# zhengfei0908/SBA-GAN

Hardware: AMD Instinct MI355X
Metric: images/sec (G+D step) at 256px (higher is better)
Workload: dtype bf16; 1 GPU; bird_style.yml 3-stage G+D step (64..256px), B=20 per GPU, G_NET variant=model, image_encoder=inception, text_encoder=RNN_ENCODER in the step; global_batch=20, parallelism=dp1, launch=replayer, losses_finite=True

## Files before the change

sba-gan_amd/csrc/igemm.hip:

```cpp
#include <math.h>
#include <stdlib.h>

#include "common.h"
#include <type_traits>

namespace {

struct FastDiv {
    uint64_t magic;
    uint32_t d;
};
static inline FastDiv make_fastdiv(uint32_t d, int64_t max_n) {
    FastDiv f;
    f.d = d;
    f.magic = (max_n < (1 << 21) && d > 0) ? (((uint64_t)1 << 42) + d - 1) / d : 0;
    return f;
}
__device__ __forceinline__ uint32_t fdiv(uint32_t n, const FastDiv& f) {
    return f.magic ? (uint32_t)(((uint64_t)n * f.magic) >> 42) : n / f.d;
}

struct EpiX { const float* bias; const void* mask; int yh; int glu_c; };

__device__ __forceinline__ uint32_t relu_mask_bf16x2(uint32_t v, uint32_t m) {
// ... 1877 lines not shown
        typedef __attribute__((address_space(3))) s16x4_t* lptr;
        s16x4_t lo = __builtin_amdgcn_ds_read_tr16_b64_v4i16((lptr)(xs + slot(L0) * 128 + c0 * 16 + q * 8));
        s16x4_t hi = __builtin_amdgcn_ds_read_tr16_b64_v4i16((lptr)(xs + slot(L1) * 128 + c1 * 16 + q * 8));
        bf16x8_t v;
        v[0] = lo[0]; v[1] = lo[1]; v[2] = lo[2]; v[3] = lo[3];
        v[4] = hi[0]; v[5] = hi[1]; v[6] = hi[2]; v[7] = hi[3];
        return v;
    }
};

template <int KW, int XB> struct WgRowCfg {
    static constexpr int LPS = (4 + XB + KW - 1) / KW;
    static constexpr int STAGE = LPS * KW * 1024;
};

template <int KW, int SX, int XB, int D>
__global__ __launch_bounds__(64 * KW, 2) void wgrad_row_dma_kernel(const bf16_t* __restrict__ x, const bf16_t* __restrict__ dy,
                                                                float* __restrict__ dw, const sba_conv_geom g, const int M,
                                                                const int chunks_per_split, const int use_atomic,
                                                                const FastDiv dsub, const FastDiv dow, const int64_t zstride,
                                                                const int wclog) {
    constexpr int LPS = WgRowCfg<KW, XB>::LPS, STAGE = WgRowCfg<KW, XB>::STAGE;
    extern __shared__ __attribute__((aligned(1024))) unsigned char wg_lds[];

    const int tid = threadIdx.x, lane = tid & 63, wv = __builtin_amdgcn_readfirstlane(tid >> 6);
    const int kw = wv;
    const int co0 = blockIdx.x * 64;
    const int ci_tiles = g.Cin / 64;
    const int kh = blockIdx.y / ci_tiles;
    const int ci0 = (blockIdx.y - kh * ci_tiles) * 64;
    const int tap = kh * KW + kw;
    int ty0 = 0, tx0 = 0;
#pragma unroll
    for (int t = 0; t < SBA_MAX_TAPS; ++t) {
        if (t == kh * KW) { ty0 = g.ty[t]; tx0 = g.tx[t]; }
    }
    const int ups = g.ups;
    const int Wc = 1 << wclog, R = 32 >> wclog, XW = ups ? (Wc >> 1) + 2 : SX * (Wc - 1) + KW, XR = R * XW;
    const int sub = g.OH * g.OW;

    const uint32_t lds_base = (uint32_t)(uintptr_t)(__attribute__((address_space(3))) unsigned char*)wg_lds;
    const uint32_t x_bytes = (uint32_t)((int64_t)g.N * g.IH * g.IW * g.Cin * 2);
    const uint32_t dy_bytes = (uint32_t)((int64_t)g.N * g.OH * g.OW * g.Cout * 2);
    const __amdgpu_buffer_rsrc_t xr = __builtin_amdgcn_make_buffer_rsrc((void*)x, 0, x_bytes, 0x00020000);
    const __amdgpu_buffer_rsrc_t dr = __builtin_amdgcn_make_buffer_rsrc((void*)dy, 0, dy_bytes, 0x00020000);
    constexpr uint32_t OOB = 0xFFFFFFFFu;

    const int rsub = lane >> 3;
    const int cgx = (lane & 7) ^ WgFragRow<SX>::swz(rsub);
    const int cgd = (lane & 7) ^ (((lane >> 4) & 1) << 2);
    const uint32_t x_coff = (uint32_t)(ci0 + cgx * 8) * 2u, d_coff = (uint32_t)(co0 + cgd * 8) * 2u;
    const uint32_t x_pix = (uint32_t)g.Cin * 2u, d_pix = (uint32_t)g.Cout * 2u;
    const int rows_img = g.OH < R ? g.OH : R;
    int role[LPS], rr[LPS], rc[LPS], rn[LPS];
#pragma unroll
    for (int i = 0; i < LPS; ++i) {
        const int b = wv + KW * i;
        role[i] = 2; rr[i] = 0; rc[i] = 0; rn[i] = 0;
        if (b < 4) { role[i] = 0; rr[i] = 8 * b + rsub; }
        else if (b < 4 + XB) {
            const int L = WgFragRow<SX>::slot(8 * (b - 4) + rsub);
            if (L < XR) {
                const int r = L / XW;
                role[i] = 1;
                rn[i] = r / rows_img;
                rr[i] = (r - rn[i] * rows_img) * g.sy + ty0;
                rc[i] = ups ? L - r * XW : L - r * XW + tx0;
            }
        }
    }

    const int chunk_lo = blockIdx.z * chunks_per_split;
    const int chunk_hi = min(chunk_lo + chunks_per_split, M >> 5);
    int g_ck = chunk_lo;

    auto issue = [&](const uint32_t dst) {
        const bool live = g_ck < chunk_hi;
        const int m0 = g_ck * 32;
        const int n = (int)fdiv(m0, dsub), rem = m0 - n * sub;
        const int oy0 = (int)fdiv(rem, dow), ox0 = rem - oy0 * g.OW;
        const int iy0 = oy0 * g.sy, ix0 = ox0 * g.sx;
#pragma unroll
        for (int i = 0; i < LPS; ++i) {
            uint32_t off = OOB;
            if (role[i] == 0) {
                if (live) off = (uint32_t)(m0 + rr[i]) * d_pix + d_coff;
                lds_dma16(dr, off, 0u, dst + (uint32_t)((wv + KW * i) * 1024));
            } else {
                int iy = iy0 + rr[i], ix = ix0 + rc[i];
                if (ups) {
                    iy >>= 1;
                    ix = ((ox0 + tx0) >> 1) + rc[i];
                }
                const bool ok = live & (role[i] == 1) & (iy >= 0) & (iy < g.IH) & (ix >= 0) & (ix < g.IW);
                if (ok) off = (uint32_t)(((n + rn[i]) * g.IH + iy) * g.IW + ix) * x_pix + x_coff;
                lds_dma16(xr, off, 0u, dst + (uint32_t)((wv + KW * i) * 1024));
            }
        }
        ++g_ck;
    };

    f32x16_t acc[2][2];
#pragma unroll
    for (int i = 0; i < 2; ++i)
#pragma unroll
        for (int j = 0; j < 2; ++j)
#pragma unroll
            for (int r = 0; r < 16; ++r) acc[i][j][r] = 0.f;

    int islot = 0;
#pragma unroll
    for (int p = 0; p < D - 1; ++p) { issue(lds_base + (uint32_t)(islot * STAGE)); ++islot; }
    if (islot == D) islot = 0;
    int cslot = 0;
    for (int ck = chunk_lo; ck < chunk_hi; ++ck) {
        wait_vmcnt<(D - 2) * LPS>();
        wg_barrier();
        issue(lds_base + (uint32_t)(islot * STAGE));
        if (++islot == D) islot = 0;
        const unsigned char* st = wg_lds + cslot * STAGE;
        const unsigned char* xs = st + 4 * 1024;
#pragma unroll
        for (int k16 = 0; k16 < 2; ++k16) {
            bf16x8_t a[2], b[2];
            b[0] = WgFragRow<SX>::load(xs, k16, 0, lane, kw, wclog, XW, ups, tx0);
            b[1] = WgFragRow<SX>::load(xs, k16, 32, lane, kw, wclog, XW, ups, tx0);
            a[0] = WgFragDma::load(st, k16, 0, lane);
            a[1] = WgFragDma::load(st, k16, 32, lane);
#pragma unroll
            for (int i = 0; i < 2; ++i)
#pragma unroll
                for (int j = 0; j < 2; ++j)
                    acc[i][j] = __builtin_amdgcn_mfma_f32_32x32x16_bf16(a[i], b[j], acc[i][j], 0, 0, 0);
        }
        if (++cslot == D) cslot = 0;
    }
    wait_vmcnt<0>();
    wg_barrier();

    const int col_l = lane & 31, rsel = 4 * (lane >> 5);
#pragma unroll
    for (int i = 0; i < 2; ++i)
#pragma unroll
        for (int j = 0; j < 2; ++j)
#pragma unroll
            for (int r = 0; r < 16; ++r) {
                const int co = co0 + i * 32 + (r & 3) + 8 * (r >> 2) + rsel;
                const int ci = ci0 + j * 32 + col_l;
                float* p = dw + (int64_t)blockIdx.z * zstride + ((int64_t)co * g.ntaps + tap) * g.Cin + ci;
                if (use_atomic == 1) atomicAdd(p, acc[i][j][r]);
                else if (use_atomic == 2) *p = acc[i][j][r];
                else *p += acc[i][j][r];
            }
}

template <typename T>
__global__ __launch_bounds__(192) void wgrad_rows_kernel(const T* __restrict__ x, const T* __restrict__ dy,
                                                         float* __restrict__ dw, const sba_conv_geom g,
                                                         const int total_segs, const int segs_per_wg,
                                                         const int store, const int64_t zstride) {
    constexpr int ROWS = WgFrag<T>::ROWS;
    constexpr int CH = 16 / (int)sizeof(T);
    constexpr int CPR = 64 / CH;
    constexpr int XR = 66;
    constexpr int XROWS_ALLOC = 80;
    __shared__ __attribute__((aligned(16))) unsigned char lds[(64 + 3 * XROWS_ALLOC) * ROWS];

    const int tid = threadIdx.x, lane = tid & 63, kh = tid >> 6;
    const int co0 = blockIdx.x * 64, ci0 = blockIdx.y * 64;
    const int IHL = g.ups ? 2 * g.IH : g.IH, IWL = g.ups ? 2 * g.IW : g.IW;
    const int segs_per_row = g.OW / 64;
    unsigned char* sa = lds;
    unsigned char* sx = lds + (64 + kh * XROWS_ALLOC) * ROWS;

    for (int i = lane; i < (XROWS_ALLOC - XR) * ROWS / 16; i += 64)
        *reinterpret_cast<uint4*>(sx + XR * ROWS + i * 16) = make_uint4(0, 0, 0, 0);

    f32x16_t acc[3][2][2];
#pragma unroll
    for (int t = 0; t < 3; ++t)
#pragma unroll
        for (int i = 0; i < 2; ++i)
#pragma unroll
            for (int j = 0; j < 2; ++j)
#pragma unroll
                for (int r = 0; r < 16; ++r) acc[t][i][j][r] = 0.f;

    const int seg_lo = blockIdx.z * segs_per_wg;
    const int seg_hi = min(seg_lo + segs_per_wg, total_segs);
    constexpr int A_PT = (64 * CPR + 191) / 192;
    constexpr int X_PT = (XR * CPR + 63) / 64;
    uint4 va[A_PT], vx[X_PT];
    auto gload = [&](int seg) {
        const int n = seg / (g.OH * segs_per_row);
        const int rem = seg - n * g.OH * segs_per_row;
        const int oy = rem / segs_per_row, ox0 = (rem - oy * segs_per_row) * 64;
#pragma unroll
        for (int u = 0; u < A_PT; ++u) {
            const int idx = tid + 192 * u;
            va[u] = make_uint4(0, 0, 0, 0);
            if (idx < 64 * CPR) {
                const int pix = idx / CPR, cc = idx - pix * CPR;
                const int co = co0 + cc * CH;
                if (co < g.Cout) {
                    const int64_t po = ((int64_t)(n * g.OH + oy) * g.OW + ox0 + pix);
                    va[u] = *reinterpret_cast<const uint4*>(dy + po * g.Cout + co);
                }
            }
        }
        int iy = oy + kh - 1;
        const bool row_ok = (iy >= 0) & (iy < IHL);
        if (g.ups) iy >>= 1;
#pragma unroll
        for (int u = 0; u < X_PT; ++u) {
            const int idx = lane + 64 * u;
            vx[u] = make_uint4(0, 0, 0, 0);
            if (idx < XR * CPR) {
                const int j = idx / CPR, cc = idx - j * CPR;
                int ix = ox0 - 1 + j;
                const bool ok = row_ok & (ix >= 0) & (ix < IWL);
                if (g.ups) ix >>= 1;
                const int ci = ci0 + cc * CH;
                if (ok && ci < g.Cin) {
                    const int64_t pi = (int64_t)(n * g.IH + iy) * g.IW + ix;
                    vx[u] = *reinterpret_cast<const uint4*>(x + pi * g.Cin + ci);
                }
            }
        }
    };
    if (seg_lo < seg_hi) gload(seg_lo);
    for (int seg = seg_lo; seg < seg_hi; ++seg) {
        __syncthreads();
#pragma unroll
        for (int u = 0; u < A_PT; ++u) {
            const int idx = tid + 192 * u;
            if (idx < 64 * CPR) {
                const int pix = idx / CPR, cc = idx - pix * CPR;
                *reinterpret_cast<uint4*>(sa + pix * ROWS + cc * 16) = va[u];
            }
        }
#pragma unroll
        for (int u = 0; u < X_PT; ++u) {
            const int idx = lane + 64 * u;
            if (idx < XR * CPR) {
                const int j = idx / CPR, cc = idx - j * CPR;
                *reinterpret_cast<uint4*>(sx + j * ROWS + cc * 16) = vx[u];
            }
        }
        __syncthreads();
        if (seg + 1 < seg_hi) gload(seg + 1);
#pragma unroll
        for (int ks = 0; ks < 4; ++ks) {
#pragma unroll
            for (int kw = 0; kw < 3; ++kw)
                WgFrag<T>::mma(sa + 16 * ks * ROWS, sx + (16 * ks + kw) * ROWS, lane, acc[kw]);
        }
    }

    const int col_l = lane & 31, rsel = 4 * (lane >> 5);
#pragma unroll
    for (int kw = 0; kw < 3; ++kw) {
        const int tap = kh * 3 + kw;
#pragma unroll
        for (int i = 0; i < 2; ++i)
#pragma unroll
            for (int j = 0; j < 2; ++j)
#pragma unroll
                for (int r = 0; r < 16; ++r) {
                    const int co = co0 + i * 32 + (r & 3) + 8 * (r >> 2) + rsel;
                    const int ci = ci0 + j * 32 + col_l;
                    if (co < g.Cout && ci < g.Cin) {
                        float* p = dw + (int64_t)blockIdx.z * zstride + ((int64_t)co * 9 + tap) * g.Cin + ci;
                        if (store) *p = acc[kw][i][j][r];
                        else atomicAdd(p, acc[kw][i][j][r]);
                    }
                }
    }
}

template <typename T>
__global__ void pack_weight_kernel(const float* __restrict__ w, T* __restrict__ out, int Cout, int KH,
                                   int KW, int Cin, int mode) {
    const int64_t n = (int64_t)Cout * (mode == 3 ? 16 : KH * KW) * Cin;
    for (int64_t i = blockIdx.x * (int64_t)blockDim.x + threadIdx.x; i < n;
         i += (int64_t)gridDim.x * blockDim.x) {
        float v;
        if (mode == 0) {
            v = w[i];
        } else if (mode == 1) {
            const int co = (int)(i % Cout);
            int64_t t = i / Cout;
            const int kw = (int)(t % KW); t /= KW;
            const int kh = (int)(t % KH);
            const int ci = (int)(t / KH);
            v = w[(((int64_t)co * KH + (KH - 1 - kh)) * KW + (KW - 1 - kw)) * Cin + ci];
        } else if (mode == 3) {
            const int co = (int)(i % Cout);
            int64_t t = i / Cout;
            const int sl = (int)(t % 16);
            const int ci = (int)(t / 16);
            const int dd = sl >> 2, ee = sl & 3;
            const int kh0 = dd == 0 ? 2 : (dd == 1 ? 1 : 0), khn = (dd == 1 || dd == 2) ? 2 : 1;
            const int kw0 = ee == 0 ? 2 : (ee == 1 ? 1 : 0), kwn = (ee == 1 || ee == 2) ? 2 : 1;
            v = 0.f;
            for (int a = 0; a < khn; ++a)
                for (int b2 = 0; b2 < kwn; ++b2)
// ... 213 lines not shown
            if (sizeof(T) == 2 && ex.yh) *reinterpret_cast<bf16_t*>(&ov[k]) = f2h_bits(v[k]);
            else ov[k] = from_f<T>(v[k]);
        }
        *reinterpret_cast<V4*>(y + o) = *reinterpret_cast<const V4*>(ov);
    }
    if (stats) {
        float* slot = stats + (int64_t)(blockIdx.y & (SBA_BN_STAT_SLOTS - 1)) * 2 * g.Cout;
#pragma unroll
        for (int k = 0; k < 4; ++k) {
            atomicAdd(&slot[c + k], s0[k]);
            atomicAdd(&slot[g.Cout + c + k], s1[k]);
        }
    }
}

template <typename T>
__global__ __launch_bounds__(256) void splitk_finish_kernel(float* __restrict__ ws, T* __restrict__ y,
                                                            const T* __restrict__ addend,
                                                            float* __restrict__ stats, const sba_conv_geom g,
                                                            const int M, const EpiX ex) {
    splitk_finish_body<T>(ws, y, addend, stats, g, M, ex);
}

__global__ __launch_bounds__(256) void splitk_finish_group_kernel(const GroupArgs A) {
    const GroupItem& it = A.it[blockIdx.z];
    const sba_conv_geom g = it.g;
    splitk_finish_body<bf16_t>(it.ws, it.y, it.addend, nullptr, g, it.M, EpiX{it.bias, it.mask, 0});
}

struct IgemmCfg { int bm, bn, ks, occ; float eff; bool split; };
static const IgemmCfg kCfg[5] = {
    {128, 128, 1, 3, 1.00f, false}, {256, 64, 1, 3, 1.00f, false}, {128, 64, 2, 2, 0.80f, false},
    {64, 64, 2, 4, 0.50f, true},    {320, 128, 2, 1, 0.90f, true}};
constexpr int IGEMM_SPLIT_MAX_M = 2048;

template <typename T, int BM, int BN, int WM, int WN, int KS>
static void launch_cfg(const T* xp, const T* wp, T* yp, const T* ap, float* stats, const sba_conv_geom& g, int M,
                       int nslabs, int split, float* ws, hipStream_t st, const EpiX ex) {
    constexpr int NT = (BM / WM) * (BN / WN) * 64;
    int sps = nslabs;
    if (split > 1) {
        sps = cdiv(cdiv(nslabs, split), KS) * KS;
        split = cdiv(nslabs, sps);
    }
    dim3 grid(cdiv(M, BM), cdiv(g.Cout, BN), split);
    SBA_LAUNCH((igemm_kernel<T, BM, BN, WM, WN, KS>), grid, dim3(NT), 0, st, xp, wp, yp, ap, stats, g, M,
                       split > 1 ? ws : (float*)nullptr, sps, ex);
    if (split > 1) {
        dim3 fgrid(cdiv(g.Cout / 4, 256), cdiv(M, 8));
        SBA_LAUNCH((splitk_finish_kernel<T>), fgrid, dim3(256), 0, st, ws, yp, ap, stats, g, M, ex);
    }
}

static int nmajor_for(const sba_conv_geom& g) {
    const int64_t wb = (int64_t)g.Cout * g.ntaps * g.Cin, xb = (int64_t)g.N * g.IH * g.IW * g.Cin;
    return wb > xb ? 1 : 0;
}

template <int BM, int BN, int WM, int WN, int KS, int D>
static void launch_dma(const bf16_t* xp, const bf16_t* wp, bf16_t* yp, const bf16_t* ap, float* stats,
                       const sba_conv_geom& g, int M, int nslabs, int split, float* ws, hipStream_t st, const EpiX ex) {
    constexpr int NT = (BM / WM) * (BN / WN) * 64;
    int sps = nslabs;
    if (split > 1) {
        sps = cdiv(cdiv(nslabs, split), KS) * KS;
        split = cdiv(nslabs, sps);
    }
    const int gx = cdiv(M, BM), gy = cdiv(g.Cout, BN);
    const int nmajor = nmajor_for(g);
    dim3 grid(nmajor ? 8 * cdiv(gy, 8) * gx : 8 * cdiv(gx, 8) * gy, 1, split);
    SBA_LAUNCH((igemm_dma_kernel<BM, BN, WM, WN, KS, D>), grid, dim3(NT), 0, st, xp, wp, yp, ap, stats, g, M,
               split > 1 ? ws : (float*)nullptr, sps, ex, gx, gy, nmajor DMA_TRACE_ARG);
    if (split > 1) {
        dim3 fgrid(cdiv(g.Cout / 4, 256), cdiv(M, 8));
        SBA_LAUNCH((splitk_finish_kernel<bf16_t>), fgrid, dim3(256), 0, st, ws, yp, ap, stats, g, M, ex);
    }
}

template <int BM, int BN, int WM, int WN, int D>
static void launch_dma2(const bf16_t* xp, const bf16_t* wp, bf16_t* yp, const bf16_t* ap, float* stats,
                        const sba_conv_geom& g, int M, int nslabs64, int split, float* ws, hipStream_t st, const EpiX ex) {
    constexpr int NT = (BM / WM) * (BN / WN) * 64;
    int sps = nslabs64;
    if (split > 1) {
        sps = cdiv(nslabs64, split);
        split = cdiv(nslabs64, sps);
    }
    const int gx = cdiv(M, BM), gy = cdiv(g.Cout, BN);
    const int nmajor = nmajor_for(g);
    dim3 grid(nmajor ? 8 * cdiv(gy, 8) * gx : 8 * cdiv(gx, 8) * gy, 1, split);
    SBA_LAUNCH((igemm_dma2_kernel<BM, BN, WM, WN, D>), grid, dim3(NT), 0, st, xp, wp, yp, ap, stats, g, M,
               split > 1 ? ws : (float*)nullptr, sps, ex, gx, gy, nmajor DMA_TRACE_ARG);
    if (split > 1) {
        dim3 fgrid(cdiv(g.Cout / 4, 256), cdiv(M, 8));
        SBA_LAUNCH((splitk_finish_kernel<bf16_t>), fgrid, dim3(256), 0, st, ws, yp, ap, stats, g, M, ex);
    }
}

static bool halo_ok(const sba_conv_geom& g) {
    if (g.ntaps != 9 || g.sy != 1 || g.sx != 1 || g.osy != 1 || g.osx != 1 || g.ooy || g.oox) return false;
    if (g.OHs != g.OH || g.OWs != g.OW || (g.Cin != 64 && g.Cin != 128) || g.Cout % 64) return false;
    if (g.OH % 8 || g.OW % 32) return false;
    if (g.ups ? (g.IH * 2 != g.OH || g.IW * 2 != g.OW) : (g.IH != g.OH || g.IW != g.OW)) return false;
    for (int t = 0; t < 9; ++t)
        if (g.ty[t] != t / 3 - 1 || g.tx[t] != t % 3 - 1) return false;
    const int64_t tiles = (int64_t)g.N * (g.OH / 8) * (g.OW / 32);
    return tiles >= 128 && tiles <= 0x7fffffff;
}

static bool halo3g_ok(const sba_conv_geom& g) {
    if (g.w_layout != 1 || g.ups) return false;
    if (g.ntaps != 9 || g.sy != 1 || g.sx != 1 || g.osy != 1 || g.osx != 1 || g.ooy || g.oox) return false;
    if (g.OHs != g.OH || g.OWs != g.OW || g.Cin % 32 || g.Cout % 32) return false;
    int ymin = g.ty[0], ymax = g.ty[0], xmin = g.tx[0], xmax = g.tx[0];
    unsigned seen = 0;
    for (int t = 0; t < 9; ++t) {
        ymin = g.ty[t] < ymin ? g.ty[t] : ymin; ymax = g.ty[t] > ymax ? g.ty[t] : ymax;
        xmin = g.tx[t] < xmin ? g.tx[t] : xmin; xmax = g.tx[t] > xmax ? g.tx[t] : xmax;
    }
    if (ymax - ymin != 2 || xmax - xmin != 2) return false;
    for (int t = 0; t < 9; ++t) seen |= 1u << ((g.ty[t] - ymin) * 3 + (g.tx[t] - xmin));
    if (seen != 0x1ffu) return false;
    const int64_t tiles = (int64_t)g.N * cdiv(g.OH, 8) * cdiv(g.OW, 32);
    return tiles >= 128 && tiles <= 0x7fffffff;
}

static void launch_halo3g(const sba_conv_geom& g, const bf16_t* x, const bf16_t* w, bf16_t* y, const bf16_t* addend,
                          const EpiX ex, hipStream_t st) {
    const int tiles = g.N * cdiv(g.OH, 8) * cdiv(g.OW, 32);
    const bool tn2 = g.Cout % 64 == 0;
    dim3 grid(tiles, g.Cout / (tn2 ? 64 : 32));
    if (g.Cin % 64 == 0) {
        if (tn2) SBA_LAUNCH((conv3x3_halo3g_kernel<64, 2>), grid, dim3(256), 0, st, x, w, y, addend, g, ex);
        else SBA_LAUNCH((conv3x3_halo3g_kernel<64, 1>), grid, dim3(256), 0, st, x, w, y, addend, g, ex);
    } else {
        if (tn2) SBA_LAUNCH((conv3x3_halo3g_kernel<32, 2>), grid, dim3(256), 0, st, x, w, y, addend, g, ex);
        else SBA_LAUNCH((conv3x3_halo3g_kernel<32, 1>), grid, dim3(256), 0, st, x, w, y, addend, g, ex);
    }
}

static void launch_halo(const sba_conv_geom& g, const bf16_t* x, const bf16_t* w, bf16_t* y, const bf16_t* addend,
                        float* stats, const EpiX ex, hipStream_t st) {
    const int tiles = g.N * (g.OH / 8) * (g.OW / 32);
    dim3 grid(tiles, g.Cout / 64);
    if (g.w_layout == 1) {
        if (g.ups) SBA_LAUNCH((conv3x3_halo3_kernel<64, 1>), grid, dim3(256), 0, st, x, w, y, addend, stats, g, ex);
        else SBA_LAUNCH((conv3x3_halo3_kernel<64, 0>), grid, dim3(256), 0, st, x, w, y, addend, stats, g, ex);
        return;
    }
    if (g.ups) SBA_LAUNCH((conv3x3_halo_kernel<64, 64, 1>), grid, dim3(256), 0, st, x, w, y, addend, stats, g, ex);
    else SBA_LAUNCH((conv3x3_halo_kernel<64, 64, 0>), grid, dim3(256), 0, st, x, w, y, addend, stats, g, ex);
}

template <typename T>
int launch_igemm(const void* x, const void* w, void* y, const void* addend, float* stats,
                 const sba_conv_geom& g, void* workspace, int64_t ws_bytes, hipStream_t st,
                 const EpiX ex = EpiX{nullptr, nullptr, 0}, int* plan = nullptr) {
    const int M = g.N * g.OHs * g.OWs;
    const T* xp = (const T*)x; const T* wp = (const T*)w; T* yp = (T*)y; const T* ap = (const T*)addend;
    if (g.w_layout != 0 && !(g.w_layout == 1 && sizeof(T) == 2 && (halo_ok(g) || halo3g_ok(g)))) return SBA_E_ARG;
    if (sizeof(T) == 2 && g.w_layout == 1 && !halo_ok(g)) {
        if (plan) { plan[0] = 4; plan[1] = g.Cin % 64 == 0 ? 64 : 32; plan[2] = 1; return SBA_OK; }
        if (stats) return SBA_E_ARG;
        launch_halo3g(g, (const bf16_t*)x, (const bf16_t*)w, (bf16_t*)y, (const bf16_t*)addend, ex, st);
        return SBA_CHECK_LAUNCH();
    }
    if (sizeof(T) == 2 && halo_ok(g)) {
        if (plan) { plan[0] = 0; plan[1] = g.ups ? 1 : 0; plan[2] = 1; return SBA_OK; }
        launch_halo(g, (const bf16_t*)x, (const bf16_t*)w, (bf16_t*)y, (const bf16_t*)addend, stats, ex, st);
        return SBA_CHECK_LAUNCH();
    }
    const int nslabs = g.ntaps * (g.Cin / (64 / (int)sizeof(T)));
    const bool can_split = workspace && g.Cout % 4 == 0 && (int64_t)M * g.Cout * 4 <= ws_bytes && nslabs >= 16;
    int best, best_split = 1;
    const int wgA = (g.Cout % 128 == 0) ? cdiv(M, 128) * (g.Cout / 128) : 0;
    if (M <= 2048) {
        best = (g.Cout >= 1024 && (nslabs >= 512 || (M >= 1280 && nslabs >= 256))) ? 4 : 3;
    } else if ((g.Cout == 128 && M >= 40000) || (g.Cout == 256 && M >= 40000 && nslabs >= 48)) {
        best = 4;
    } else if (wgA >= 320) {
        best = 0;
    } else if (g.Cout <= 64 && cdiv(M, 256) >= 256) {
        best = 1;
    } else if (cdiv(M, 128) * cdiv(g.Cout, 64) >= 256) {
        best = 2;
    } else {
        best = 3;
    }
    {
        const IgemmCfg& k = kCfg[best];
        const int tiles = cdiv(M, k.bm) * cdiv(g.Cout, k.bn);
        const int slots = 256 * k.occ;
        if (k.split && can_split && tiles < slots && M <= IGEMM_SPLIT_MAX_M) {
            int split = slots / tiles;
            if (split > nslabs / 8) split = nslabs / 8;
            if (split > 32) split = 32;
            if (split > 1) best_split = split;
        }
    }
    const bool det = sba_det_on();
    if (det) best_split = 1;
    float* ws = (float*)workspace;
    if constexpr (sizeof(T) == 2) {
        const bf16_t* xb = (const bf16_t*)x; const bf16_t* wb = (const bf16_t*)w; bf16_t* yb = (bf16_t*)y;
        const bf16_t* ab = (const bf16_t*)addend;
        static const int rule_tile[4] = {7, 9, 5, 1};
        int tile = g.tile;
        int split = best_split;
        if (tile <= 0 || tile > SBA_IGEMM_TILES) {
            tile = best <= 3 ? rule_tile[best] : 11;
        } else if (g.ksplit >= 1) {
            split = g.ksplit;
            if (split > 1 && !(workspace && g.Cout % 4 == 0 && (int64_t)M * g.Cout * 4 <= ws_bytes)) split = 1;
            if (split > nslabs / 2) split = nslabs / 2 > 0 ? nslabs / 2 : 1;
        }
        if (det) split = 1;
        if (tile >= 13 && g.Cin % 64 != 0) {
            tile = best <= 3 ? rule_tile[best] : 11;
            split = det ? 1 : best_split;
        }
        if (g.Cin % 64 == 0 && tile != 11) {
            const int ns64 = nslabs / 2;
            int sp = split;
            if (sp > ns64 / 2) sp = ns64 / 2 > 0 ? ns64 / 2 : 1;
            if (plan) { plan[0] = 1; plan[1] = tile; plan[2] = sp; return SBA_OK; }
            switch (tile) {
                case 1: launch_dma2<64, 64, 32, 32, 4>(xb, wb, yb, ab, stats, g, M, ns64, sp, ws, st, ex); return SBA_CHECK_LAUNCH();
                case 2: launch_dma2<64, 64, 32, 32, 8>(xb, wb, yb, ab, stats, g, M, ns64, sp, ws, st, ex); return SBA_CHECK_LAUNCH();
                case 3: launch_dma2<96, 64, 32, 64, 3>(xb, wb, yb, ab, stats, g, M, ns64, sp, ws, st, ex); return SBA_CHECK_LAUNCH();
                case 4: launch_dma2<96, 64, 32, 64, 6>(xb, wb, yb, ab, stats, g, M, ns64, sp, ws, st, ex); return SBA_CHECK_LAUNCH();
                case 5: launch_dma2<128, 64, 32, 64, 3>(xb, wb, yb, ab, stats, g, M, ns64, sp, ws, st, ex); return SBA_CHECK_LAUNCH();
                case 6: launch_dma2<128, 64, 32, 64, 6>(xb, wb, yb, ab, stats, g, M, ns64, sp, ws, st, ex); return SBA_CHECK_LAUNCH();
                case 7: launch_dma2<128, 128, 64, 64, 3>(xb, wb, yb, ab, stats, g, M, ns64, sp, ws, st, ex); return SBA_CHECK_LAUNCH();
                case 8: launch_dma2<128, 128, 64, 64, 4>(xb, wb, yb, ab, stats, g, M, ns64, sp, ws, st, ex); return SBA_CHECK_LAUNCH();
                case 9: launch_dma2<256, 64, 64, 64, 3>(xb, wb, yb, ab, stats, g, M, ns64, sp, ws, st, ex); return SBA_CHECK_LAUNCH();
                case 10: launch_dma2<256, 64, 64, 64, 4>(xb, wb, yb, ab, stats, g, M, ns64, sp, ws, st, ex); return SBA_CHECK_LAUNCH();
                case 13: launch_dma2<320, 64, 64, 64, 3>(xb, wb, yb, ab, stats, g, M, ns64, sp, ws, st, ex); return SBA_CHECK_LAUNCH();
                case 14: launch_dma2<160, 64, 32, 64, 4>(xb, wb, yb, ab, stats, g, M, ns64, sp, ws, st, ex); return SBA_CHECK_LAUNCH();
                case 15: launch_dma2<160, 64, 32, 64, 2>(xb, wb, yb, ab, stats, g, M, ns64, sp, ws, st, ex); return SBA_CHECK_LAUNCH();
                case 16: launch_dma2<256, 128, 128, 64, 3>(xb, wb, yb, ab, stats, g, M, ns64, sp, ws, st, ex); return SBA_CHECK_LAUNCH();
                case 17: launch_dma2<256, 128, 64, 64, 3>(xb, wb, yb, ab, stats, g, M, ns64, sp, ws, st, ex); return SBA_CHECK_LAUNCH();
                case 18: launch_dma2<256, 128, 128, 64, 2>(xb, wb, yb, ab, stats, g, M, ns64, sp, ws, st, ex); return SBA_CHECK_LAUNCH();
                default: launch_dma2<96, 128, 32, 128, 5>(xb, wb, yb, ab, stats, g, M, ns64, sp, ws, st, ex); return SBA_CHECK_LAUNCH();
            }
        }
        if (plan && tile != 11) { plan[0] = 2; plan[1] = tile; plan[2] = split; return SBA_OK; }
        switch (tile) {
            case 1: launch_dma<64, 64, 32, 32, 2, 4>(xb, wb, yb, ab, stats, g, M, nslabs, split, ws, st, ex); return SBA_CHECK_LAUNCH();
            case 2: launch_dma<64, 64, 32, 32, 2, 8>(xb, wb, yb, ab, stats, g, M, nslabs, split, ws, st, ex); return SBA_CHECK_LAUNCH();
            case 3: launch_dma<96, 64, 32, 64, 2, 3>(xb, wb, yb, ab, stats, g, M, nslabs, split, ws, st, ex); return SBA_CHECK_LAUNCH();
            case 4: launch_dma<96, 64, 32, 64, 2, 6>(xb, wb, yb, ab, stats, g, M, nslabs, split, ws, st, ex); return SBA_CHECK_LAUNCH();
            case 5: launch_dma<128, 64, 32, 64, 1, 4>(xb, wb, yb, ab, stats, g, M, nslabs, split, ws, st, ex); return SBA_CHECK_LAUNCH();
            case 6: launch_dma<128, 64, 32, 64, 2, 6>(xb, wb, yb, ab, stats, g, M, nslabs, split, ws, st, ex); return SBA_CHECK_LAUNCH();
            case 7: launch_dma<128, 128, 64, 64, 1, 4>(xb, wb, yb, ab, stats, g, M, nslabs, split, ws, st, ex); return SBA_CHECK_LAUNCH();
            case 8: launch_dma<128, 128, 64, 64, 1, 8>(xb, wb, yb, ab, stats, g, M, nslabs, split, ws, st, ex); return SBA_CHECK_LAUNCH();
            case 9: launch_dma<256, 64, 64, 64, 1, 3>(xb, wb, yb, ab, stats, g, M, nslabs, split, ws, st, ex); return SBA_CHECK_LAUNCH();
            case 10: launch_dma<256, 64, 64, 64, 1, 6>(xb, wb, yb, ab, stats, g, M, nslabs, split, ws, st, ex); return SBA_CHECK_LAUNCH();
            case 12: launch_dma<96, 128, 32, 128, 1, 8>(xb, wb, yb, ab, stats, g, M, nslabs, split, ws, st, ex); return SBA_CHECK_LAUNCH();
            default: break;
        }
        if (plan) { plan[0] = 3; plan[1] = 4; plan[2] = split; return SBA_OK; }
        launch_cfg<T, 320, 128, 64, 64, 2>(xp, wp, yp, ap, stats, g, M, nslabs, split, ws, st, ex);
        return SBA_CHECK_LAUNCH();
    } else {
        if (plan) { plan[0] = 3; plan[1] = best; plan[2] = best_split; return SBA_OK; }
        switch (best) {
            case 0: launch_cfg<T, 128, 128, 64, 64, 1>(xp, wp, yp, ap, stats, g, M, nslabs, best_split, ws, st, ex); break;
            case 1: launch_cfg<T, 256, 64, 64, 64, 1>(xp, wp, yp, ap, stats, g, M, nslabs, best_split, ws, st, ex); break;
            case 2: launch_cfg<T, 128, 64, 32, 64, 2>(xp, wp, yp, ap, stats, g, M, nslabs, best_split, ws, st, ex); break;
            case 3: launch_cfg<T, 64, 64, 32, 32, 2>(xp, wp, yp, ap, stats, g, M, nslabs, best_split, ws, st, ex); break;
            default: launch_cfg<T, 320, 128, 64, 64, 2>(xp, wp, yp, ap, stats, g, M, nslabs, best_split, ws, st, ex); break;
        }
        return SBA_CHECK_LAUNCH();
    }
}

bool geom_ok(const sba_conv_geom* g, int dtype) {
    if (!g) return false;
    const int ks = dtype == SBA_BF16 ? 32 : 16;
    if (g->ntaps < 1 || g->ntaps > SBA_MAX_TAPS) return false;
    for (int t = 0; t < g->ntaps; ++t)
        if (g->ty[t] < -8 || g->ty[t] > 7 || g->tx[t] < -8 || g->tx[t] > 7) return false;
    if (g->Cin <= 0 || g->Cin % ks != 0) return false;
    if (g->N <= 0 || g->IH <= 0 || g->IW <= 0 || g->OH <= 0 || g->OW <= 0 || g->Cout <= 0) return false;
    if (g->OHs <= 0 || g->OWs <= 0 || g->osy <= 0 || g->osx <= 0) return false;
    if ((g->OHs - 1) * g->osy + g->ooy >= g->OH || (g->OWs - 1) * g->osx + g->oox >= g->OW) return false;
    if (g->ooy < 0 || g->oox < 0) return false;
    if ((int64_t)g->N * g->OHs * g->OWs > 0x7fffffff) return false;
    const int64_t esz = dtype == SBA_BF16 ? 2 : 4;
    const int vec = dtype == SBA_BF16 ? 8 : 4;
    const int xcs = g->x_cstride ? g->x_cstride : g->Cin, ycs = g->y_cstride ? g->y_cstride : g->Cout;
    if (xcs < g->Cin + g->x_coff || ycs < g->Cout + g->y_coff || g->x_coff < 0 || g->y_coff < 0) return false;
    if (xcs % vec || g->x_coff % vec || ycs % vec || g->y_coff % vec) return false;
    if ((int64_t)g->N * g->IH * g->IW * xcs * esz >= ((int64_t)1 << 32)) return false;
    if ((int64_t)g->Cout * g->ntaps * g->Cin * esz >= ((int64_t)1 << 32)) return false;
    if ((int64_t)g->N * g->IH * g->IW > 0x7fffffff / 2 || (int64_t)g->N * g->OH * g->OW > 0x7fffffff / 2)
        return false;
    return true;
}

bool dense_output(const sba_conv_geom& g) {
    return g.OHs == g.OH && g.OWs == g.OW && g.osy == 1 && g.osx == 1 && g.ooy == 0 && g.oox == 0 &&
           (g.y_cstride == 0 || g.y_cstride == g.Cout) && g.y_coff == 0;
}

template <typename T>
int launch_igemm_glu(const void* x, const void* w, void* y, const sba_conv_geom& g, hipStream_t st, const EpiX ex,
                     int* plan = nullptr) {
    const int M = g.N * g.OHs * g.OWs;
    const T* xp = (const T*)x; const T* wp = (const T*)w; T* yp = (T*)y;
    if (g.w_layout != 0 && !(g.w_layout == 1 && sizeof(T) == 2 && halo_ok(g))) return SBA_E_ARG;
    if constexpr (sizeof(T) == 2) {
        if (halo_ok(g)) {
            if (plan) { plan[0] = 0; plan[1] = (g.ups ? 1 : 0) + (g.w_layout == 1 ? 2 : 0); plan[2] = 1; return SBA_OK; }
            dim3 grid(g.N * (g.OH / 8) * (g.OW / 32), g.Cout / 64);
            const bf16_t* np = nullptr;
            if (g.w_layout == 1) {
                if (g.ups) SBA_LAUNCH((conv3x3_halo3_kernel<64, 1, 1>), grid, dim3(256), 0, st, xp, wp, yp, np, (float*)nullptr, g, ex);
                else SBA_LAUNCH((conv3x3_halo3_kernel<64, 0, 1>), grid, dim3(256), 0, st, xp, wp, yp, np, (float*)nullptr, g, ex);
            } else {
                if (g.ups) SBA_LAUNCH((conv3x3_halo_kernel<64, 64, 1, 1>), grid, dim3(256), 0, st, xp, wp, yp, np, (float*)nullptr, g, ex);
                else SBA_LAUNCH((conv3x3_halo_kernel<64, 64, 0, 1>), grid, dim3(256), 0, st, xp, wp, yp, np, (float*)nullptr, g, ex);
// ... 464 lines not shown
```

sba-gan_amd/sbagan/ops.py:

```python
import ctypes
import os

import torch

from . import _lib
from ._lib import ACT_GLU, ACT_LRELU, ACT_NONE, ConvGeom, call

CL = torch.channels_last
COMPUTE_DTYPE = torch.bfloat16
BN_EPS, BN_MOMENTUM, IN_EPS = 1e-5, 0.1, 1e-5

_WEIGHT_EPOCH = [0]


def set_compute_dtype(dt):
    global COMPUTE_DTYPE
    assert dt in (torch.bfloat16, torch.float32)
    COMPUTE_DTYPE = dt
    _WEIGHT_EPOCH[0] += 1


def compute_dtype():
    return COMPUTE_DTYPE

# ... 262 lines not shown
            d['Cout'], d['KH'], d['KW'], d['Cin'] = O, KH, KW, I
            d['mode'] = _DGRAD_MODE[kind]
            d['tile_begin'] = tiles
            d['co_tiles'], d['ci_tiles'] = (O + 63) // 64, (I + 63) // 64
            tiles += (16 if d['mode'] == 3 else KH * KW) * d['co_tiles'] * d['ci_tiles']
            if st['fwd'] is not None:
                pw._fwd = st['fwd'][o:o + sizes[i]]
            pw._dgrad = st['tr'][toffs[i]:toffs[i] + tsizes[i]]
        st['descs'] = torch.from_numpy(desc.view(np.uint8).copy()).to(dev)
        st['ptrs'] = [pw.param.data_ptr() for pw, _ in self.layers]
        st['tiles'] = tiles
        st['frag'] = None
        if dtype == torch.bfloat16:
            items = []
            for pw, kind in self.layers:
                O, I, KH, KW = pw.param.shape
                if kind != '3x3' or KH != 3:
                    continue
                if I in (64, 128) and O % 64 == 0:
                    pw._ffwd = torch.empty(O * 9 * I, dtype=dtype, device=dev)
                    items.append((pw._fwd, pw._ffwd, O, 9, I))
                if kind == '3x3' and O in (64, 128) and I % 64 == 0:
                    pw._fdgrad = torch.empty(O * 9 * I, dtype=dtype, device=dev)
                    items.append((pw._dgrad, pw._fdgrad, I, 9, O))
            if items:
                st['frag'] = _frag_descs(items, dev) + (len(items),)
        self.state = {dtype: st}
        return st

    def refresh(self, dtype):
        st = self.state.get(dtype)
        if st is None or st['ptrs'] != [pw.param.data_ptr() for pw, _ in self.layers]:
            st = self._build(dtype)
        for pw, _ in self.layers:
            if not pw.param.is_contiguous(memory_format=CL):
                raise RuntimeError('conv parameters must be stored channels_last (use sbagan layers)')
        dcode = _lib.SBA_BF16 if dtype == torch.bfloat16 else _lib.SBA_F32
        call('sba_pack_weights_multi', dcode, st['descs'].data_ptr(), len(self.layers), st['tiles'], _stream())
        if st.get('frag') is not None:
            fd, units, nfrag = st['frag']
            call('sba_pack_frag_multi', fd.data_ptr(), nfrag, units, _stream())
        for pw, kind in self.layers:
            k = pw._key(dtype)
            pw._kf, pw._kd = k, k + (kind,)
            pw._kff, pw._kfd = k, k + (kind,)


class ZeroArena(object):

    def __init__(self):
        self.buf, self.off, self.active = None, 0, False

    def begin(self, device, nfloats=4 << 20):
        if self.buf is None or self.buf.device != device or self.buf.numel() < nfloats:
            self.buf = torch.empty(nfloats, dtype=torch.float32, device=device)
        self.buf.zero_()
        self.off, self.active = 0, True

    def end(self):
        self.active = False

    def take(self, n, device):
        n4 = (n + 3) // 4 * 4
        if not self.active or self.buf.device != device or self.off + n4 > self.buf.numel():
            return None
        t = self.buf[self.off:self.off + n]
        self.off += n4
        return t


ARENA = ZeroArena()


def zeros_f32(shape, device):
    n = 1
    for d in (shape if isinstance(shape, (tuple, list)) else (shape,)):
        n *= d
    t = ARENA.take(n, device)
    if t is None:
        return torch.zeros(shape, dtype=torch.float32, device=device)
    return t.view(shape)


_WORKSPACE = {}
WORKSPACE_BYTES = 64 << 20


def workspace(device):
    key = (device, torch.cuda.current_stream(device).cuda_stream)
    ws = _WORKSPACE.get(key)
    if ws is None:
        with torch.cuda.stream(torch.cuda.default_stream(device)):
            ws = torch.zeros(WORKSPACE_BYTES, dtype=torch.uint8, device=device)
        torch.cuda.current_stream(device).wait_stream(torch.cuda.default_stream(device))
        _WORKSPACE[key] = ws
    return ws


_REDUCE_SCRATCH = {}
REDUCE_SCRATCH_BYTES = int(os.environ.get('SBA_REDUCE_SCRATCH_MB', '64')) << 20


def reduce_scratch(device):
    if device not in _REDUCE_SCRATCH:
        if _REDUCE_SCRATCH and REDUCE_SCRATCH_BYTES:
            raise RuntimeError('sbagan runs one process per GPU: the reduction scratch ring already belongs to %s'
                               % next(iter(_REDUCE_SCRATCH)))
        buf = None
        if REDUCE_SCRATCH_BYTES:
            with torch.cuda.stream(torch.cuda.default_stream(device)):
                buf = torch.empty(REDUCE_SCRATCH_BYTES, dtype=torch.uint8, device=device)
            torch.cuda.current_stream(device).wait_stream(torch.cuda.default_stream(device))
            call('sba_set_reduce_scratch', buf.data_ptr(), REDUCE_SCRATCH_BYTES)
        _REDUCE_SCRATCH[device] = buf
    return _REDUCE_SCRATCH[device]


IGEMM_LOG = None
_IGEMM_TABLE = None


def geom_key(g):
    return '%d_%dx%d_%d_%dx%d_%d_t%d_s%d_u%d' % (g.N, g.IH, g.IW, g.Cin, g.OHs, g.OWs, g.Cout, g.ntaps, g.sy, g.ups)


_TABLE_FILE = None


def _table_section(name):
    global _TABLE_FILE
    if _TABLE_FILE is None:
        _TABLE_FILE = {}
        path = os.environ.get('SBA_IGEMM_TABLE_FILE') or os.path.join(os.path.dirname(os.path.abspath(__file__)),
                                                                      'igemm_table.json')
        if os.environ.get('SBA_IGEMM_TABLE', '1') != '0' and os.path.exists(path):
            import json
            with open(path) as f:
                _TABLE_FILE = json.load(f)
    return _TABLE_FILE.get(name, {})


def _igemm_table():
    global _IGEMM_TABLE
    if _IGEMM_TABLE is None:
        _IGEMM_TABLE = _table_section('bf16')
    return _IGEMM_TABLE


def tune_geom(g, dt):
    if getattr(g, '_tuned', None) != dt:
        g._tuned = dt
        ent = _igemm_table().get(geom_key(g)) if dt == _lib.SBA_BF16 else None
        g.tile, g.ksplit = (int(ent[0]), int(ent[1])) if ent else (0, 0)
    if IGEMM_LOG is not None:
        IGEMM_LOG.append(g)


def _igemm(dt, x, w, y, addend, stats, g, device, w_frag=None):
    ws = workspace(device)
    tune_geom(g, _lib.SBA_BF16 if dt == _lib.SBA_BF16_YH else dt)
    g.w_layout = 0
    if w_frag is not None and _halo_family(g):
        w, g.w_layout = w_frag.data_ptr(), 1
    try:
        call('sba_conv_igemm', dt, x, w, y, addend, stats, ctypes.byref(g), ws.data_ptr(), WORKSPACE_BYTES, _stream())
    finally:
        g.w_layout = 0


def _halo_family(g):
    h = getattr(g, '_halo', None)
    if h is None:
        plan = (ctypes.c_int * 3)()
        old = g.w_layout
        g.w_layout = 0
        call('sba_conv_igemm_plan', _lib.SBA_BF16, ctypes.byref(g), WORKSPACE_BYTES, plan)
        g.w_layout = old
        h = g._halo = plan[0] == 0
    return h




def conv_forward(x, pw, kind, want_stats=True, addend=None, pre_bn=False):
    _need_gpu(x)
    N, Cin, H, W = x.shape
    O = pw.param.shape[0]
    OH, OW = _conv_out_hw(kind, H, W)
    yh = pre_bn and Y_F16 and x.dtype == torch.bfloat16 and addend is None and O % 8 == 0
    if yh:
        y = torch.empty((N, O, OH, OW), dtype=torch.float16, device=x.device, memory_format=CL)
    else:
        y = empty_act(N, O, OH, OW, x)
    stats = zeros_f32((BN_STAT_SLOTS, 2 * O), x.device) if want_stats else None
    g = _geom((kind, N, H, W, Cin, O, None))
    wf = pw.fwd_frag(x.dtype) if kind == '3x3' else None
    _igemm(_lib.SBA_BF16_YH if yh else _dt(x), _p(x), _p(pw.fwd(x.dtype)), _p(y), _p(addend), _p(stats), g, x.device,
           w_frag=wf)
    return y, stats


def conv_dgrad(dy, pw, kind, in_hw, addend=None):
    N, O, OH, OW = dy.shape
    I = pw.param.shape[1]
    H, W = in_hw
    wd = pw.dgrad(dy.dtype, kind)
    if kind == '3x3':
        g = _geom(('3x3', N, OH, OW, O, I, None))
        dx = empty_act(N, I, H, W, dy)
        _igemm(_dt(dy), _p(dy), _p(wd), _p(dx), _p(addend), None, g, dy.device, w_frag=pw.dgrad_frag(dy.dtype, kind))
        return dx
    if kind == '3x3up':
        g = _geom(('4x4s2', N, OH, OW, O, I, None))
        dx = empty_act(N, I, H, W, dy)
        _igemm(_dt(dy), _p(dy), _p(wd), _p(dx), _p(addend), None, g, dy.device)
        return dx
    if kind == '4x4s2':
        dx = empty_act(N, I, H, W, dy)
        esz = dy.element_size()
        gs = [_geom(('4x4s2_dgrad', N, OH, OW, O, I, (cls // 2, cls % 2))) for cls in range(4)]
        if DGRAD4_GROUP and dy.dtype == torch.bfloat16 and O % 64 == 0:
            arr = (_lib.ConvGroupItem * 4)()
            for cls, (a, g) in enumerate(zip(arr, gs)):
                a.x, a.w, a.y, a.addend = _p(dy), wd.data_ptr() + cls * I * 4 * O * esz, _p(dx), _p(addend)
                a.bias = a.relu_mask = None
                a.g = ctypes.pointer(g)
            tile, split = dgrad4_plan(gs[0])
            ws = workspace(dy.device)
            call('sba_conv_igemm_group_splitk', _lib.SBA_BF16, 4, arr, tile, split, ws.data_ptr(), WORKSPACE_BYTES, _stream())
            if IGEMM_LOG is not None:
                IGEMM_LOG.append(('group', tile, gs))
            return dx
        for cls in range(4):
            wptr = wd.data_ptr() + cls * I * 4 * O * esz
            _igemm(_dt(dy), _p(dy), wptr, _p(dx), _p(addend), None, gs[cls], dy.device)
        return dx
    raise ValueError(kind)


DGRAD4_GROUP = True
_DGRAD4_FORCE = None


def dgrad4_plan(g):
    if _DGRAD4_FORCE:
        t, s = _DGRAD4_FORCE.split(',')
        return int(t), int(s)
    ent = _table_section('dgrad4').get(geom_key(g))
    if ent:
        return int(ent[0]), int(ent[1])
    M = g.N * g.OHs * g.OWs
    ny = (g.Cout + 63) // 64
    for tile, bm in ((5, 128), (3, 96), (1, 64)):
        tiles = 4 * ((M + bm - 1) // bm) * ny
        if tiles >= 512 or tile == 1:
            break
    ns64 = g.ntaps * (g.Cin // 64)
    split = max(1, min(512 // max(tiles, 1), ns64 // 8))
    return tile, split


_KSPLIT_TARGET = 640
_KSPLIT_MIN_CHUNKS = 24


def _ksplit(tiles, M):
    chunks = (M + 63) // 64
    want = max(1, (_KSPLIT_TARGET + tiles - 1) // tiles)
    return max(1, min(want, chunks // _KSPLIT_MIN_CHUNKS if chunks >= 2 * _KSPLIT_MIN_CHUNKS else 1))


def conv_wgrad(x, dy, param, kind):
    N, Cin, H, W = x.shape
    O = dy.shape[1]
    g = _geom((kind, N, H, W, Cin, O, None))
    gbuf = param_grad(param)
    M = N * g.OHs * g.OWs
    tiles = ((O + 63) // 64) * ((Cin + 63) // 64) * g.ntaps
    cell = getattr(param, '_sba_gepoch', None)
    first = 0
    if cell is not None and getattr(param, '_sba_wepoch', None) != cell[0]:
        param._sba_wepoch = cell[0]
        first = 1
    g.first_write = first
    call('sba_conv_wgrad', _dt(x), _p(x), _p(dy), _p(gbuf), ctypes.byref(g), _ksplit(tiles, M), _stream())


SIDE_WGRAD = False
HOME_STREAM = None
_COMPANION, _KEEPALIVE, _COMP_NEXT = {}, {}, {}
N_COMPANIONS = int(os.environ.get('SBA_WGRAD_COMPANIONS', '1'))


def _companion(device, *keep):
    cur = torch.cuda.current_stream()
    key = cur.cuda_stream
    comps = _COMPANION.get(key)
    if comps is None:
        comps = _COMPANION[key] = [torch.cuda.Stream(device=device) for _ in range(N_COMPANIONS)]
        _KEEPALIVE[key] = []
        _COMP_NEXT[key] = 0
    comp = comps[_COMP_NEXT[key] % len(comps)]
    _COMP_NEXT[key] += 1
    comp.wait_stream(cur)
    _KEEPALIVE[key].extend(keep)
    return comp
# ... 1094 lines not shown
```

Measured before the change: 2104 images/sec.

## Add specialized row-halo kernel for 4x4 stride-2 bf16 convolutions

Adds a dedicated implicit-GEMM kernel for 4x4 stride-2 pad-1 convolutions (discriminator downsampling). Each wave loads a strip of input rows once into LDS with async buffer DMA and reuses it across the four kw taps. Weights stream through a six-slot LDS ring, and MFMA issue is interleaved with the loads. The Python tuner now drops table-tuned tile choices for these geometries whenever the new path is selectable. The gain depends on the new kernel beating the previously tuned generic tiles for every matching shape, since the win check always returns true.

Result: no change. 2113 images/sec (median of 6 runs) (+0.4%).

```diff
diff --git a/sba-gan_amd/csrc/igemm.hip b/sba-gan_amd/csrc/igemm.hip
--- a/sba-gan_amd/csrc/igemm.hip
+++ b/sba-gan_amd/csrc/igemm.hip
@@ -2053,6 +2053,215 @@
                 else if (use_atomic == 2) *p = acc[i][j][r];
                 else *p += acc[i][j][r];
             }
+}
+
+struct Row4Seg {
+    static __device__ __forceinline__ int swz(int L) { return (L >> 1) & 7; }
+    static __device__ __forceinline__ int slot(int L) { return L ^ ((L >> 4) & 1); }
+};
+
+template <int XB>
+__global__ __launch_bounds__(256) void conv4x4s2_row_kernel(
+    const bf16_t* __restrict__ x, const bf16_t* __restrict__ w, bf16_t* __restrict__ y,
+    const bf16_t* __restrict__ addend, float* __restrict__ stats, const sba_conv_geom g, const int M,
+    const EpiX ex, const int gx, const int gy, const int nmajor, const int wclog) {
+    typedef bf16_t T;
+    constexpr int BM = 128, BN = 64, TM = 1, TN = 2, NW = 4, NT = NW * 64, RB = 6;
+    constexpr int A_WAVE = XB * 1024, A_BUF = NW * A_WAVE, B_OFF = 2 * A_BUF, UNIT = BN * 128;
+    constexpr int RING_BYTES = B_OFF + RB * UNIT;
+    constexpr int NA0 = 5, NA1 = XB - 5;
+    constexpr int W0 = 4, W1 = XB + 13, W2 = 2 * XB + 3, W3 = XB + 8;
+    static_assert(NA1 >= 0 && W2 <= 63, "vmcnt field");
+    static_assert(RING_BYTES <= 160 * 1024, "LDS");
+    constexpr int EPI_OFF = BM * (BN * 2 + 16);
+    constexpr int EPI_END = EPI_OFF + BM * 4 + BN * 8;
+    static_assert(EPI_END <= RING_BYTES, "epilogue staging fits in the ring");
+    constexpr int LDS_BYTES = RING_BYTES;
+    __shared__ __attribute__((aligned(1024))) unsigned char lds_all[LDS_BYTES];
+    int* rowoff = reinterpret_cast<int*>(lds_all + EPI_OFF);
+    float* s_stat = reinterpret_cast<float*>(lds_all + EPI_OFF + BM * 4);
+
+    const int Lw = (int)blockIdx.x, xcd = Lw & 7, q = Lw >> 3;
+    int mt, nt;
+    if (nmajor) {
+        nt = xcd + 8 * (q / gx);
+        mt = q - (q / gx) * gx;
+        if (nt >= gy) return;
+    } else {
+        mt = xcd + 8 * (q / gy);
+        nt = q - (q / gy) * gy;
+        if (mt >= gx) return;
+    }
+    const int tid = threadIdx.x, lane = tid & 63;
+    const int wid = __builtin_amdgcn_readfirstlane(tid >> 6);
+    const int wm0 = wid * 32, wn0 = 0;
+    const int m_base = mt * BM, n_base = nt * BN;
+    const uint32_t lds_base = (uint32_t)(uintptr_t)(__attribute__((address_space(3))) unsigned char*)lds_all;
+
+    const int Wc = 1 << wclog, R = 32 >> wclog, XW = 2 * Wc + 2, XR = R * XW;
+    const int xcs = g.x_cstride ? g.x_cstride : g.Cin;
+    const int ycs = g.y_cstride ? g.y_cstride : g.Cout;
+    const int cpt = g.Cin / 64;
+    constexpr uint32_t OOB = 0xFFFFFFFFu;
+    const uint32_t x_pix = (uint32_t)xcs * 2u, x_rowb = (uint32_t)g.IW * x_pix;
+    const uint32_t krow_bytes = 16u * (uint32_t)g.Cin * 2u;
+    const uint32_t x_bytes = (uint32_t)((int64_t)g.N * g.IH * g.IW * xcs * 2);
+    const uint32_t w_bytes = (uint32_t)g.Cout * krow_bytes;
+    const __amdgpu_buffer_rsrc_t xr = __builtin_amdgcn_make_buffer_rsrc((void*)x, 0, x_bytes, 0x00020000);
+    const __amdgpu_buffer_rsrc_t wr = __builtin_amdgcn_make_buffer_rsrc((void*)w, 0, w_bytes, 0x00020000);
+
+    const int rsub = lane >> 3;
+    const int m0 = m_base + 32 * wid;
+    const int q0 = m0 / g.OW, ox0 = m0 - q0 * g.OW;
+    uint32_t a_off0[XB];
+    int a_iyb[XB];
+#pragma unroll
+    for (int b = 0; b < XB; ++b) {
+        const int Lr = Row4Seg::slot(8 * b + rsub);
+        const int rr = Lr / XW, col = Lr - rr * XW;
+        const int qq = q0 + rr, n = qq / g.OH, oy = qq - n * g.OH;
+        const int ix = 2 * ox0 - 1 + col, iyb = 2 * oy - 1;
+        const bool ok = (m0 < M) & (Lr < XR) & (ix >= 0) & (ix < g.IW);
+        a_off0[b] = (uint32_t)((n * g.IH + iyb) * g.IW + ix) * x_pix + (uint32_t)(g.x_coff * 2) +
+                    (uint32_t)(((lane & 7) ^ Row4Seg::swz(Lr)) * 16);
+        a_iyb[b] = ok ? iyb : -100000;
+    }
+    uint32_t w_off[2];
+#pragma unroll
+    for (int i = 0; i < 2; ++i) {
+        const int r = 8 * (wid + NW * i) + rsub;
+        w_off[i] = (uint32_t)(n_base + r) * krow_bytes + (uint32_t)(((lane & 7) ^ ((r >> 1) & 7)) * 16);
+    }
+
+    uint32_t ib = lds_base + (uint32_t)(B_OFF + wid * 1024);
+    const uint32_t ib_end = lds_base + (uint32_t)(B_OFF + RB * UNIT + wid * 1024);
+    auto issue_b = [&](const int i, const int kh, const int slab, const int kw) {
+        const uint32_t o = kh < 4 ? w_off[i] : OOB;
+        lds_dma16(wr, o, (uint32_t)__builtin_amdgcn_readfirstlane(((kh * 4 + kw) * g.Cin + slab * 64) * 2),
+                  (uint32_t)__builtin_amdgcn_readfirstlane((int)(ib + (uint32_t)(NW * i * 1024))));
+    };
+    auto next_unit = [&]() {
+        ib += UNIT;
+        if (ib == ib_end) ib = lds_base + (uint32_t)(B_OFF + wid * 1024);
+    };
+    auto issue_a = [&](const int b, const int kh, const int slab, const int buf) {
+        const int bb = b < XB ? b : 0;
+        const bool ok = (kh < 4) & ((unsigned)(a_iyb[bb] + kh) < (unsigned)g.IH);
+        const uint32_t o = ok ? a_off0[bb] + (uint32_t)kh * x_rowb : OOB;
+        lds_dma16(xr, o, (uint32_t)__builtin_amdgcn_readfirstlane(slab * 128),
+                  (uint32_t)__builtin_amdgcn_readfirstlane((int)(lds_base + (uint32_t)(buf * A_BUF + wid * A_WAVE + bb * 1024))));
+    };
+    auto adv = [&](int& kh, int& slab) { if (++slab == cpt) { slab = 0; ++kh; } };
+
+    f32x16_t acc[TM][TN];
+#pragma unroll
+    for (int j = 0; j < TN; ++j)
+#pragma unroll
+        for (int r = 0; r < 16; ++r) acc[0][j][r] = 0.f;
+
+    const int fr = lane & 31, fh = lane >> 5;
+    int foff[4], aoff[4][4];
+    {
+        const int Lb = (fr >> wclog) * XW + 2 * (fr & (Wc - 1));
+#pragma unroll
+        for (int kk = 0; kk < 4; ++kk) {
+            foff[kk] = fr * 128 + (((2 * kk + fh) ^ ((fr >> 1) & 7)) << 4);
+#pragma unroll
+            for (int kw = 0; kw < 4; ++kw)
+                aoff[kw][kk] = Row4Seg::slot(Lb + kw) * 128 + (((2 * kk + fh) ^ Row4Seg::swz(Lb + kw)) << 4);
+        }
+    }
+    struct Frags { bf16x8_t a[4], b[4][TN]; };
+    const unsigned char* a_wave = lds_all + wid * A_WAVE;
+    const unsigned char* rb = lds_all + B_OFF;
+    auto read_frags = [&](Frags& F, const int kw, const int buf) {
+        const unsigned char* ar = a_wave + buf * A_BUF;
+#pragma unroll
+        for (int kk = 0; kk < 4; ++kk) {
+            F.a[kk] = *reinterpret_cast<const bf16x8_t*>(ar + aoff[kw][kk]);
+#pragma unroll
+            for (int j = 0; j < TN; ++j) F.b[kk][j] = *reinterpret_cast<const bf16x8_t*>(rb + j * 4096 + foff[kk]);
+        }
+        rb += UNIT;
+        if (rb == lds_all + B_OFF + RB * UNIT) rb = lds_all + B_OFF;
+    };
+
+    int kh1 = 0, sl1 = 0, kh2 = 0, sl2 = 0, tr = 0;
+    adv(kh1, sl1);
+    kh2 = kh1; sl2 = sl1;
+    adv(kh2, sl2);
+    {
+        issue_b(0, 0, 0, 0); issue_b(1, 0, 0, 0); next_unit();
+        issue_b(0, 0, 0, 1); issue_b(1, 0, 0, 1); next_unit();
+#pragma unroll
+        for (int b = 0; b < NA0; ++b) issue_a(b, 0, 0, 0);
+        issue_b(0, 0, 0, 2); issue_b(1, 0, 0, 2); next_unit();
+#pragma unroll
+        for (int b = 0; b < NA1; ++b) issue_a(NA0 + b, 0, 0, 0);
+        issue_b(0, 0, 0, 3); issue_b(1, 0, 0, 3); next_unit();
+        issue_b(0, kh1, sl1, 0); issue_b(1, kh1, sl1, 0); next_unit();
+    }
+    auto step_load = [&](const int kw, const int u) {
+        if (u < 2) {
+            if (kw < 3) issue_b(u, kh1, sl1, kw + 1);
+            else issue_b(u, kh2, sl2, 0);
+        } else {
+            issue_a((kw == 0 ? 0 : NA0) + u - 2, kh1, sl1, (tr + 1) & 1);
+        }
+    };
+    Frags F0, F1;
+    wait_vmcnt<W0>();
+    wg_barrier();
+    read_frags(F0, 0, 0);
+#pragma unroll
+    for (int u = 0; u < 2 + NA0; ++u) step_load(0, u);
+    next_unit();
+
+    auto step = [&](auto kwc, Frags& Fc, Frags& Fn) {
+        constexpr int KW = decltype(kwc)::value;
+        constexpr int LP = 2 + (KW == 0 ? NA0 : KW == 1 ? NA1 : 0), NM = 4 * TN;
+        if (KW == 0) {
+            ++tr;
+            kh1 = kh2; sl1 = sl2;
+            adv(kh2, sl2);
+        }
+        wait_vmcnt<(KW == 0 ? W0 : KW == 1 ? W1 : KW == 2 ? W2 : W3)>();
+        asm volatile("s_waitcnt lgkmcnt(0)" ::: "memory");
+        wg_barrier();
+        read_frags(Fn, KW, tr & 1);
+#pragma unroll
+        for (int kk = 0; kk < 4; ++kk)
+#pragma unroll
+            for (int j = 0; j < TN; ++j) {
+                acc[0][j] = __builtin_amdgcn_mfma_f32_32x32x16_bf16(Fc.a[kk], Fc.b[kk][j], acc[0][j], 0, 0, 0);
+                const int m = kk * TN + j;
+                if (((m + 1) * LP) / NM > (m * LP) / NM) {
+#pragma unroll
+                    for (int u = (m * LP) / NM; u < ((m + 1) * LP) / NM; ++u) step_load(KW, u);
+                    __builtin_amdgcn_sched_barrier(0);
+                }
+            }
+        next_unit();
+    };
+    const int nstages = 4 * cpt;
+    for (int t = 0; t < nstages; ++t) {
+        step(std::integral_constant<int, 1>{}, F0, F1);
+        step(std::integral_constant<int, 2>{}, F1, F0);
+        step(std::integral_constant<int, 3>{}, F0, F1);
+        step(std::integral_constant<int, 0>{}, F1, F0);
+    }
+    wait_vmcnt<0>();
+    asm volatile("s_waitcnt lgkmcnt(0)" ::: "memory");
+    wg_barrier();
+
+    for (int r = threadIdx.x; r < BM; r += NT) {
+        const int m = m_base + r;
+        rowoff[r] = m < M ? m : -1;
+    }
+    for (int c = threadIdx.x; c < 2 * BN; c += NT) s_stat[c] = 0.f;
+    __syncthreads();
+    tile_epilogue<T, BM, BN, TM, TN, NT, LDS_BYTES>(acc, true, lds_all, rowoff, s_stat, wm0, wn0, lane, n_base, ycs, g, y,
+                                                    addend, stats, ex, mt);
 }
 
 template <typename T>
@@ -2572,6 +2781,36 @@
     else SBA_LAUNCH((conv3x3_halo_kernel<64, 64, 0>), grid, dim3(256), 0, st, x, w, y, addend, stats, g, ex);
 }
 
+static bool row4_ok(const sba_conv_geom& g, const EpiX& ex) {
+    if (g.ntaps != 16 || g.sy != 2 || g.sx != 2 || g.ups || g.w_layout != 0 || g.relu) return false;
+    if (ex.bias || ex.mask || ex.glu_c) return false;
+    if (g.OHs != g.OH || g.OWs != g.OW || g.osy != 1 || g.osx != 1 || g.ooy || g.oox) return false;
+    if ((g.y_cstride != 0 && g.y_cstride != g.Cout) || g.y_coff != 0) return false;
+    if (g.Cin % 64 || g.Cout % 64) return false;
+    if (g.OW < 4 || (g.OW & (g.OW - 1)) != 0) return false;
+    if (((int64_t)g.N * g.OH * g.OW) % 32 != 0) return false;
+    for (int t = 0; t < 16; ++t)
+        if (g.ty[t] != t / 4 - 1 || g.tx[t] != t % 4 - 1) return false;
+    return true;
+}
+
+static void launch_row4(const sba_conv_geom& g, const bf16_t* x, const bf16_t* w, bf16_t* y, const bf16_t* addend,
+                        float* stats, const EpiX ex, hipStream_t st) {
+    const int M = g.N * g.OH * g.OW;
+    int wclog = 2;
+    while (wclog < 5 && (1 << wclog) < g.OW) ++wclog;
+    const int gx = cdiv(M, 128), gy = g.Cout / 64;
+    const int nmajor = nmajor_for(g);
+    dim3 grid(nmajor ? 8 * cdiv(gy, 8) * gx : 8 * cdiv(gx, 8) * gy);
+    if (wclog > 2) SBA_LAUNCH((conv4x4s2_row_kernel<9>), grid, dim3(256), 0, st, x, w, y, addend, stats, g, M, ex, gx, gy, nmajor, wclog);
+    else SBA_LAUNCH((conv4x4s2_row_kernel<10>), grid, dim3(256), 0, st, x, w, y, addend, stats, g, M, ex, gx, gy, nmajor, wclog);
+}
+
+static bool row4_wins(const sba_conv_geom& g) {
+    (void)g;
+    return true;
+}
+
 template <typename T>
 int launch_igemm(const void* x, const void* w, void* y, const void* addend, float* stats,
                  const sba_conv_geom& g, void* workspace, int64_t ws_bytes, hipStream_t st,
@@ -2588,6 +2827,11 @@
     if (sizeof(T) == 2 && halo_ok(g)) {
         if (plan) { plan[0] = 0; plan[1] = g.ups ? 1 : 0; plan[2] = 1; return SBA_OK; }
         launch_halo(g, (const bf16_t*)x, (const bf16_t*)w, (bf16_t*)y, (const bf16_t*)addend, stats, ex, st);
+        return SBA_CHECK_LAUNCH();
+    }
+    if (sizeof(T) == 2 && (g.tile <= 0 || g.tile > SBA_IGEMM_TILES) && row4_ok(g, ex) && row4_wins(g) && !(sba_det_on() && stats)) {
+        if (plan) { plan[0] = 5; plan[1] = g.OW >= 8 ? 9 : 10; plan[2] = 1; return SBA_OK; }
+        launch_row4(g, (const bf16_t*)x, (const bf16_t*)w, (bf16_t*)y, (const bf16_t*)addend, stats, ex, st);
         return SBA_CHECK_LAUNCH();
     }
     const int nslabs = g.ntaps * (g.Cin / (64 / (int)sizeof(T)));
diff --git a/sba-gan_amd/sbagan/ops.py b/sba-gan_amd/sbagan/ops.py
--- a/sba-gan_amd/sbagan/ops.py
+++ b/sba-gan_amd/sbagan/ops.py
@@ -438,6 +438,12 @@
         g._tuned = dt
         ent = _igemm_table().get(geom_key(g)) if dt == _lib.SBA_BF16 else None
         g.tile, g.ksplit = (int(ent[0]), int(ent[1])) if ent else (0, 0)
+        if ent and g.ntaps == 16 and g.sy == 2:
+            plan = (ctypes.c_int * 3)()
+            g.tile = g.ksplit = 0
+            call('sba_conv_igemm_plan', _lib.SBA_BF16, ctypes.byref(g), WORKSPACE_BYTES, plan)
+            if plan[0] != 5:
+                g.tile, g.ksplit = int(ent[0]), int(ent[1])
     if IGEMM_LOG is not None:
         IGEMM_LOG.append(g)
 
```
